# TariAgentBenchmark/unet-embroidery-seg

Measured on AMD Instinct MI355X. Metric: images/sec training unet_resnet50 512×512 bf16 at 1/2/4/8 GPUs; mIoU parity, higher is better.
Workload: dtype bf16; 1 GPU; unet_resnet50 binary seg 512x512, per-GPU batch 16, lovasz_hinge + Adam; global_batch=16, image_size=512, parallelism=dp1

## Files before the change

unet-embroidery-seg_amd/csrc/conv_fast.hip:

```cpp
#include <cstdlib>
#include <type_traits>

#include "common.h"
#include "conv_fast.h"
#include "fast_util.h"


namespace {


template <int BM, int BN, int NWM, int NWN, int ST = 3>
constexpr int tn_waves_per_simd() {
  return ST == 5 ? (BN == 64 ? 4 : 3) : (BM == 64 || (BM == 128 && BN == 64)) ? 3 : 2;
}

template <int BM, int NWM, int NWN>
constexpr int kHaloChunks() {
  constexpr int NT = 64 * NWM * NWN;
  return ((BM / 32 + 2) * 34 * 8 + 2 * NT - 1) / (2 * NT) * (2 * NT);
}
template <int BM, int BN, int NWM, int NWN, int ST, int HA = 0>
constexpr size_t kPreOff() {
  constexpr size_t stages = HA ? ((size_t)2 * kHaloChunks<BM, NWM, NWN>() + (size_t)(ST - 10) * BN * 8) * 16
                               : (size_t)(ST == 1 || ST == 5 ? 1 : ST >= 13 ? ST - 10 : 2) * (BM + BN) * 8 * 16;
// ... 615 lines not shown
  constexpr int CPR = WTN / 8;
  constexpr int RPI = 64 / CPR;
  const int ck = lane % CPR, rsub = lane / CPR;
  const int nc = n0 + wn * WTN + ck * 8;
  constexpr int NQ3 = POST == 3 ? 8 : 1;
  float q3[3][NQ3], mu3[2][NQ3], iv3[2][NQ3];
  const bool two = POST == 3 && a.aux2 != nullptr;
  if constexpr (POST == 3) {
#pragma unroll
    for (int e = 0; e < 8; ++e) {
      const bool ok = nc + e < a.Ng;
      q3[0][e] = q3[1][e] = q3[2][e] = 0.f;
      mu3[0][e] = ok ? a.pmean[nc + e] : 0.f;
      iv3[0][e] = ok ? a.pinv[nc + e] : 0.f;
      mu3[1][e] = (ok && two) ? a.pmean2[nc + e] : 0.f;
      iv3[1][e] = (ok && two) ? a.pinv2[nc + e] : 0.f;
    }
  }
  constexpr int NIT = WTM / RPI;
  constexpr int GRP = (POST == 3 && NIT > 4) ? 4 : NIT;
  static_assert(NIT % GRP == 0, "row groups");
#pragma unroll
  for (int g0 = 0; g0 < NIT; g0 += GRP) {
    uint4 oldv[GRP], zv[POST == 3 ? GRP : 1], z2v[POST == 3 ? GRP : 1];
    unsigned mkv[POST == 3 ? GRP : 1];
    if (POST == 3 || a.accumulate) {
      const bf16* aux2p = two ? (const bf16*)a.aux2 : (const bf16*)a.aux;
      const long ld2 = two ? a.ld_aux2 : a.ld_aux;
      const int ncl = nc < a.Ng ? nc : a.Ng - 8;
#pragma unroll
      for (int j = 0; j < GRP; ++j) {
        const int r = (g0 + j) * RPI + rsub;
        const long opx = out_pix(r < cnt ? row0 + r : min(row0, a.M - 1));
        oldv[j] = *reinterpret_cast<const uint4*>((const bf16*)a.y + opx * a.ldy + ncl);
        if constexpr (POST == 3) {
          zv[j] = *reinterpret_cast<const uint4*>((const bf16*)a.aux + opx * a.ld_aux + ncl);
          z2v[j] = *reinterpret_cast<const uint4*>(aux2p + opx * ld2 + ncl);
          mkv[j] = (unsigned)a.mbits[opx * (a.Ng >> 3) + (ncl >> 3)];
        }
      }
    }
#pragma unroll
    for (int j = 0; j < GRP; ++j) {
      const int r = (g0 + j) * RPI + rsub;
      if (r >= cnt || nc >= a.Ng) continue;
      const long opx = out_pix(row0 + r);
      bf16* ptr = (bf16*)a.y + opx * a.ldy + nc;
      uint4 v = *reinterpret_cast<const uint4*>(tl + r * LROW + ck * 16);
      if constexpr (POST == 3) {
        const uint4 old = oldv[j], z = zv[j], z2 = z2v[j];
        const unsigned mk = mkv[j];
        const bf16* ob = reinterpret_cast<const bf16*>(&old);
        const bf16* zb = reinterpret_cast<const bf16*>(&z);
        const bf16* z2b = reinterpret_cast<const bf16*>(&z2);
        bf16* nv = reinterpret_cast<bf16*>(&v);
#pragma unroll
        for (int e = 0; e < 8; ++e) {
          const bf16 sm = (bf16)((float)nv[e] + (float)ob[e]);
          const float d = ((mk >> e) & 1u) ? (float)sm : 0.f;
          nv[e] = (bf16)d;
          q3[0][e] += d;
          q3[1][e] = fmaf(d, ((float)zb[e] - mu3[0][e]) * iv3[0][e], q3[1][e]);
          if (two) q3[2][e] = fmaf(d, ((float)z2b[e] - mu3[1][e]) * iv3[1][e], q3[2][e]);
        }
      } else if (a.accumulate) {
        const uint4 old = oldv[j];
        const bf16* ob = reinterpret_cast<const bf16*>(&old);
        bf16* nv = reinterpret_cast<bf16*>(&v);
#pragma unroll
        for (int e = 0; e < 8; ++e) nv[e] = (bf16)((float)nv[e] + (float)ob[e]);
      }
      *reinterpret_cast<uint4*>(ptr) = v;
    }
  }
  if constexpr (POST == 3) {
#pragma unroll
    for (int q = 0; q < 3; ++q)
#pragma unroll
      for (int e = 0; e < 8; ++e)
        for (int o = CPR; o < 64; o <<= 1) q3[q][e] += __shfl_xor(q3[q][e], o, 64);
    if (rsub == 0) {
#pragma unroll
      for (int e = 0; e < 8; ++e) {
        const int col = wn * WTN + ck * 8 + e;
        red[wm * BN + col] = q3[0][e];
        red[(NWM + wm) * BN + col] = q3[1][e];
        red[(2 * NWM + wm) * BN + col] = q3[2][e];
      }
    }
  }
  if (POST) {
    const int nq = (POST == 3 && a.aux2) ? 3 : 2;
    asm volatile("s_waitcnt lgkmcnt(0)\n\ts_barrier" ::: "memory");
    for (int col = tid; col < BN; col += NT) {
      const int n = n0 + col;
      if (n >= a.Ng) continue;
      float t0 = 0.f, t1 = 0.f, t2 = 0.f;
#pragma unroll
      for (int w = 0; w < NWM; ++w) {
        t0 += red[w * BN + col];
        t1 += red[(NWM + w) * BN + col];
        if (POST == 3) t2 += red[(2 * NWM + w) * BN + col];
      }
      a.ppart[(long)tile_m * nq * a.Ng + n] = t0;
      a.ppart[(long)tile_m * nq * a.Ng + a.Ng + n] = t1;
      if (nq == 3) a.ppart[(long)tile_m * nq * a.Ng + 2 * a.Ng + n] = t2;
    }
  }
  if (a.stats) {
    asm volatile("s_waitcnt lgkmcnt(0)\n\ts_barrier" ::: "memory");
    for (int col = tid; col < BN; col += NT) {
      const int n = n0 + col;
      if (n >= a.Ng) continue;
      float st = 0.f, nt = 0.f;
#pragma unroll
      for (int w = 0; w < NWM; ++w) {
        st += red[w * BN + col];
        nt += (float)max(0, min(WTM, a.M - (m0 + w * WTM)));
      }
      const float mean = st / fmaxf(nt, 1.f);
      float q = 0.f;
#pragma unroll
      for (int w = 0; w < NWM; ++w) {
        const float nw = (float)max(0, min(WTM, a.M - (m0 + w * WTM)));
        if (nw > 0.f) {
          const float d = red[w * BN + col] / nw - mean;
          q += red[(NWM + w) * BN + col] + nw * d * d;
        }
      }
      a.stats[(long)tile_m * 2 * a.Ng + n] = st;
      a.stats[(long)tile_m * 2 * a.Ng + a.Ng + n] = q;
    }
  }
}

template <int BM, int BN, int NWM, int NWN, int ST, int POST, int TAPS = 0, bool PRE = false, int HA = 0>
__global__ __launch_bounds__(64 * NWM * NWN, (tn_waves_per_simd<BM, BN, NWM, NWN, ST>())) void tn_fast_kernel(FastTNArgs a) {
  tn_fast_body<BM, BN, NWM, NWN, ST, POST, TAPS, PRE, HA>(a, blockIdx.x + gridDim.x * blockIdx.y, gridDim.x, gridDim.y);
}

struct TNMulti {
  FastTNArgs c[4];
  int start[5];
  int gx[4], gy[4];
  int n;
};

template <int BM, int BN, int NWM, int NWN, int ST, int POST>
__global__ __launch_bounds__(64 * NWM * NWN, (tn_waves_per_simd<BM, BN, NWM, NWN>())) void tn_multi_kernel(TNMulti m) {
  const int b = blockIdx.x;
  int k = 0;
  while (k + 1 < m.n && b >= m.start[k + 1]) ++k;
  tn_fast_body<BM, BN, NWM, NWN, ST, POST, 0, false>(m.c[k], b - m.start[k], m.gx[k], m.gy[k]);
}

template <int BN, int NWN>
constexpr size_t kPersistLds() {
  constexpr int HST = kHaloChunks<256, 4, NWN>();
  return (size_t)2 * HST * 16 + (size_t)3 * BN * 8 * 16 + (size_t)2 * 4 * BN * 4;
}

template <int BN, int NWN, int POST, int HA>
__global__ __launch_bounds__(512, 2) void tn_halo_persist_kernel(FastTNArgs a, int T, int ntiles, unsigned y_bytes) {
  constexpr int BM = 256, NWM = 4, NT = 512, NS = 3;
  constexpr int WTN = BN / NWN, FP = 4, FC = WTN / 16;
  constexpr int RSTEP = NT / 8;
  constexpr int B_PER = BN / RSTEP;
  static_assert(B_PER == 1 || B_PER == 2, "weight rows per thread");
  constexpr int HST = kHaloChunks<BM, NWM, NWN>();
  constexpr int HI = HST / NT;
  constexpr int HPIX = 10 * 34;
  constexpr int WST = BN * 8;
  constexpr int WP = B_PER;
  constexpr int HPC = HI / HA, TPER = 9 / HA;
  static_assert(HI % (2 * HA) == 0 && 9 % HA == 0, "halo pieces of whole instruction pairs");
  constexpr int NST = FC * FP;
  static_assert(WP + 2 * HPC + NST + 2 <= 63, "vmcnt range");
  extern __shared__ __attribute__((aligned(16))) uint4 lds[];

  const int tid = threadIdx.x, lane = tid & 63;
  const int wid = __builtin_amdgcn_readfirstlane(tid >> 6);
  const int wm = wid / NWN, wn = wid % NWN;
  const int kv = tid & 7, rb = tid >> 3;
  const int kg = lane >> 4, j16 = lane & 15;
  const int gy = (a.Ng + BN - 1) / BN;
  const int tpr = a.wc >> 5;
  const int nch = a.cin >> 6;

  const unsigned hbase = lds_addr(lds);
  const unsigned wbase = hbase + 2u * HST * 16u;
  float* red = reinterpret_cast<float*>(reinterpret_cast<char*>(lds) + 2 * HST * 16 + 3 * WST * 16);
  float* xco = red + 2 * NWM * BN;
  const bool has_bias = a.bias != nullptr;
  if (has_bias)
    for (int c = tid; c < a.Ng; c += NT) xco[c] = a.bias[c];
  if (POST && a.post == 2)
    for (int c = tid; c < a.Ng; c += NT) {
      xco[c] = a.psc[c];
      xco[a.Ng + c] = a.psh[c];
      xco[2 * a.Ng + c] = a.pmean[c];
      xco[3 * a.Ng + c] = a.pinv[c];
    }
  __syncthreads();

  const int nbk = gridDim.x, b = blockIdx.x;
  const int xq = nbk >> 3, xr = nbk & 7, xcd = b & 7;
  const int lb = (xcd < xr ? xcd * (xq + 1) : xr * (xq + 1) + (xcd - xr) * xq) + (b >> 3);
  const int tfirst = lb * T;
  const int tcount = max(0, min(T, ntiles - tfirst));

  const unsigned pb1 = a.x1_bytes / (unsigned)a.ldc1b;
  const unsigned pb2 = a.x2 ? a.x2_bytes / (unsigned)a.ldc2b : 0u;
  const unsigned pbad = (pb1 > pb2 ? pb1 : pb2) + 1u;
  const unsigned hsw = (unsigned)(((lane & 7) ^ ((lane >> 3) & 7)) * 16);
  const int kvs16 = (kv ^ ((rb >> 1) & 7)) * 16;
  struct Tile {
    int tm, n0, nb, h0, w0;
  };
  auto tile_of = [&](int j) -> Tile {
    const int tl = tfirst + j;
    Tile t;
    t.tm = tl / gy;
    t.n0 = (tl - t.tm * gy) * BN;
    const int rest = t.tm / tpr, twi = t.tm - rest * tpr;
    const int hg = rest * 8;
    t.nb = hg / a.hc;
    t.h0 = hg - t.nb * a.hc;
    t.w0 = twi * 32;
    return t;
  };
  auto halo_pix = [&](const Tile& t, int i) -> unsigned {
    const int hp = (i * (NWM * NWN) + wid) * 8 + (lane >> 3);
    const int hr = hp / 34, hc = hp - hr * 34;
    const int h = t.h0 - 1 + hr, w = t.w0 - 1 + hc;
    const bool ok = hp < HPIX && h >= 0 && h < a.H && w >= 0 && w < a.W;
    return ok ? (unsigned)((t.nb * a.H + h) * a.W + w) : pbad;
  };
  auto wrow = [&](const Tile& t, int i) -> unsigned {
    const int n = t.n0 + rb + RSTEP * i;
    return n < a.Ng ? (unsigned)n * (unsigned)a.ldwb + kvs16 : kOOB;
  };
  unsigned tw[9];
#pragma unroll
  for (int t = 0; t < 9; ++t) {
    const int jr = t / 3, js = t - jr * 3;
    tw[t] = (unsigned)(((a.r0 + a.rs * jr) * a.S + (a.s0 + a.ss * js)) * a.cin) * 2u;
  }
  int hq[FP];
#pragma unroll
  for (int p = 0; p < FP; ++p) hq[p] = (wm * 2 + (p >> 1) + 1) * 34 + (p & 1) * 16 + j16 + 1;
  const int chA = kg;
  unsigned foffW[2];
#pragma unroll
  for (int kk = 0; kk < 2; ++kk) {
    const int r = j16;
    foffW[kk] = (unsigned)((wn * WTN + r) * 128 + ((kk * 4 + kg) ^ ((r >> 1) & 7)) * 16);
  }
  auto issue_halo = [&](const Tile& tt, bool live, int cc, int hs, int i0, int i1) {
    const int c64 = cc * 64;
    const bool first = c64 < a.c1;
    const __amdgpu_buffer_rsrc_t rx = srd_u(first ? a.x1 : a.x2, !live ? 0u : first ? a.x1_bytes : a.x2_bytes);
    const unsigned ldcb = first ? (unsigned)a.ldc1b : (unsigned)a.ldc2b;
    const unsigned soff = __builtin_amdgcn_readfirstlane(live ? (unsigned)(first ? c64 : c64 - a.c1) * 2u : 0u);
    const unsigned sb = __builtin_amdgcn_readfirstlane(hbase + (unsigned)(hs * HST * 16) + (unsigned)(wid * 1024));
#pragma unroll
    for (int i = i0; i < i1; i += 2)
      dma16x2<NT * 16>(rx, sb + (unsigned)(i * NT * 16), __umul24(halo_pix(tt, i), ldcb) + hsw,
                       __umul24(halo_pix(tt, i + 1), ldcb) + hsw, soff);
  };
  auto issue_w = [&](const Tile& tt, bool live, int cc, int t, int stage) {
    const __amdgpu_buffer_rsrc_t rwx = srd_u(a.wt, live ? a.w_bytes : 0u);
    const unsigned wsoff = __builtin_amdgcn_readfirstlane(live ? tw[t] + (unsigned)(cc * 64) * 2u : 0u);
    const unsigned sb = __builtin_amdgcn_readfirstlane(wbase + (unsigned)(stage * WST * 16) + (unsigned)(wid * 8 * 128));
    if constexpr (B_PER == 1) {
      dma16s(rwx, sb, wrow(tt, 0), wsoff);
    } else {
      dma16x2<RSTEP * 128>(rwx, sb, wrow(tt, 0), wrow(tt, 1), wsoff);
    }
  };
  constexpr auto P_ = [](int t) { return ((((t % 9) + 9) % 9) % TPER == 0) ? HPC : 0; };

  const __amdgpu_buffer_rsrc_t ry = srd(a.y, y_bytes);
  const bool do_stats = a.stats != nullptr;
  const __amdgpu_buffer_rsrc_t raux = srd(POST ? a.aux : a.y, POST ? (unsigned)a.M * (unsigned)a.ld_aux * 2u : 0u);
  const __amdgpu_buffer_rsrc_t rq = srd(POST ? (const void*)a.ppart : do_stats ? (const void*)a.stats : a.y,
                                        (POST || do_stats) ? (unsigned)(a.M / BM) * 2u * (unsigned)a.Ng * 4u : 0u);
  const int E = NST + ((POST || do_stats) ? 2 : 0);

  if (tcount <= 0) return;
  Tile cur = tile_of(0);
  issue_halo(cur, true, 0, 0, 0, HI);
  issue_w(cur, true, 0, 0, 0);
  issue_w(cur, true, 0, 1, 1);

  int gc = 0;
  for (int j = 0; j < tcount; ++j) {
    const bool has_next = j + 1 < tcount;
    const Tile nxt = has_next ? tile_of(j + 1) : cur;
    f32x4 acc[FC][FP];
#pragma unroll
    for (int c = 0; c < FC; ++c)
#pragma unroll
      for (int p = 0; p < FP; ++p) acc[c][p] = f32x4{0.f, 0.f, 0.f, 0.f};
    uint2 zr[FC][FP];
    unsigned opix[FP];
#pragma unroll
// ... 515 lines not shown

template <int BM, int BN, int NWM, int NWN, int ST>
static int launch_tn_dma(const FastTNArgs& a, hipStream_t st) {
  switch (tn_taps(a)) {
    case 9: return a.post ? launch_tn_cfg<BM, BN, NWM, NWN, ST, true, 9>(a, st) : launch_tn_cfg<BM, BN, NWM, NWN, ST, false, 9>(a, st);
    case 1: return a.post ? launch_tn_cfg<BM, BN, NWM, NWN, ST, true, 1>(a, st) : launch_tn_cfg<BM, BN, NWM, NWN, ST, false, 1>(a, st);
    default: return a.post ? launch_tn_cfg<BM, BN, NWM, NWN, ST, true>(a, st) : launch_tn_cfg<BM, BN, NWM, NWN, ST>(a, st);
  }
}

static bool halo_a_ok(const FastTNArgs& a) {
  if (getenv("UNETSEG_TN_NO_HALO_RING") != nullptr || a.in_sc || a.nr != 3 || a.ns != 3 || a.istride != 1) return false;
  if (a.dhs * a.dhs != 1 || a.dws * a.dws != 1) return false;
  const int dh_lo = a.dhs > 0 ? a.dh0 : a.dh0 - 2, dw_lo = a.dws > 0 ? a.dw0 : a.dw0 - 2;
  if (dh_lo != -1 || dw_lo != -1) return false;
  if (a.H != a.hc || a.W != a.wc || a.hc % 8 || a.wc % 32) return false;
  return tn_taps(a) == 9;
}

static int tn_config_base(const FastTNArgs& a);

static int cu_count() {
  static int n = 0;
  if (!n) {
    int dev = 0;
    if (hipGetDevice(&dev) != hipSuccess || hipDeviceGetAttribute(&n, hipDeviceAttributeMultiprocessorCount, dev) != hipSuccess ||
        n <= 0)
      n = 256;
  }
  return n;
}
static int persist_t(const FastTNArgs& a, int bn) {
  const char* e = getenv("UNETSEG_TN_PERSIST");
  if (e && atoi(e) == 0) return 0;
  if (a.in_sc || a.post < 0 || a.post > 2 || (a.bias && a.post) || a.t2d < 0) return 0;
  if (a.ostride != 1 || a.ph || a.pw || a.OH != a.hc || a.OW != a.wc || a.M % 256) return 0;
  const size_t extra = (a.bias ? (size_t)a.Ng * 4 : 0) + (a.post == 2 ? (size_t)a.Ng * 16 : 0);
  const size_t lds = (bn == 128 ? kPersistLds<128, 2>() : kPersistLds<64, 2>()) + extra;
  if (lds > 160 * 1024) return 0;
  if ((unsigned long long)a.M * (unsigned)a.ldy * 2ull >= (unsigned long long)kOOB) return 0;
  if (a.post && (unsigned long long)a.M * (unsigned)a.ld_aux * 2ull >= (unsigned long long)kOOB) return 0;
  if (a.stats && (unsigned long long)(a.M / 256) * 2ull * a.Ng * 4ull >= (unsigned long long)kOOB) return 0;
  const char* mc = getenv("UNETSEG_TN_PERSIST_MIN_NCH");
  if (mc && (a.cin >> 6) < atoi(mc)) return 0;
  const long ntiles = (long)(a.M / 256) * ceil_div(a.Ng, bn);
  const char* ft = getenv("UNETSEG_TN_PERSIST_T");
  if (ft && atoi(ft) > 0) return atoi(ft);
  const char* r = getenv("UNETSEG_TN_PERSIST_ROUNDS");
  const int rounds = r && atoi(r) > 0 ? atoi(r) : 1;
  const char* m = getenv("UNETSEG_TN_PERSIST_MIN_T");
  const int min_t = m && atoi(m) > 0 ? atoi(m) : 2;
  const long T = (ntiles + (long)rounds * cu_count() - 1) / ((long)rounds * cu_count());
  return T >= min_t ? (int)T : 0;
}

template <int BN, int NWN, int HA>
static int launch_tn_persist(const FastTNArgs& a, hipStream_t st) {
  const int T = persist_t(a, BN);
  const size_t extra = (a.bias ? (size_t)a.Ng * 4 : 0) + (a.post == 2 ? (size_t)a.Ng * 16 : 0);
  const size_t lds = kPersistLds<BN, NWN>() + extra;
  const int ntiles = (a.M / 256) * ceil_div(a.Ng, BN);
  const int grid = ceil_div(ntiles, T);
  const unsigned y_bytes = (unsigned)((unsigned long long)a.M * (unsigned)a.ldy * 2ull);
  if (a.post) {
    static bool attr = false;
    if (!attr) {
      (void)hipFuncSetAttribute(reinterpret_cast<const void*>(&tn_halo_persist_kernel<BN, NWN, 1, HA>),
                                hipFuncAttributeMaxDynamicSharedMemorySize, 160 * 1024);
      attr = true;
    }
    hipLaunchKernelGGL((tn_halo_persist_kernel<BN, NWN, 1, HA>), dim3(grid), dim3(512), lds, st, a, T, ntiles, y_bytes);
  } else {
    static bool attr = false;
    if (!attr) {
      (void)hipFuncSetAttribute(reinterpret_cast<const void*>(&tn_halo_persist_kernel<BN, NWN, 0, HA>),
                                hipFuncAttributeMaxDynamicSharedMemorySize, 160 * 1024);
      attr = true;
    }
    hipLaunchKernelGGL((tn_halo_persist_kernel<BN, NWN, 0, HA>), dim3(grid), dim3(512), lds, st, a, T, ntiles, y_bytes);
  }
  return 0;
}

static int tn_config(const FastTNArgs& a) {
  if (a.force_cfg) return a.force_cfg;
  const int c = tn_config_base(a);
  if ((c == 7 || c == 13 || (c == 10 && !getenv("UNETSEG_TN_CFG_NO23"))) && halo_a_ok(a)) return c == 7 ? 21 : c == 13 ? 22 : 23;
  return c;
}

static int tn_config_base(const FastTNArgs& a) {
  if (const char* e = getenv("UNETSEG_TN_CFG")) {
    const int c = atoi(e);
    if (c == 21) return 7;
    if (((c >= 1 && c <= 14) || c == 19 || c == 20) && !(a.in_sc && c >= 7 && c <= 14)) return c;
  }
  static const bool no_dma_env = getenv("UNETSEG_TN_NO_DMA") != nullptr;
  const bool no_dma = no_dma_env || a.in_sc != nullptr;
  if (!a.in_sc && halo3_ok(a)) return 0;
  const int nsteps = a.nr * a.ns * (a.cin >> 6);
  static const bool no_short1 = getenv("UNETSEG_TN_NO_SHORT1") != nullptr;
  if (!no_short1 && nsteps <= 4 && (nsteps >= 2 || a.Ng <= 64)) return a.Ng <= 64 ? 20 : 19;
  if (nsteps == 1 && a.Ng > 64) return 4;
  if (a.Ng <= 64) return (!no_dma && nsteps >= 18 && tn_taps(a) == 9) ? 13 : 6;
  if (nsteps <= 4) return 3;
  const long tiles_big = (long)ceil_div(a.M, 256) * ceil_div(a.Ng, 128);
  if (tiles_big >= 256) return no_dma ? 2 : 7;
  const long tiles_mid = (long)ceil_div(a.M, 128) * ceil_div(a.Ng, 128);
  if (tiles_mid >= 256) return (!no_dma && nsteps >= 16 && tn_taps(a)) ? 10 : 3;
  return (!no_dma && nsteps >= 32) ? 9 : 5;
}

}

static int tn_cfg_bm(int cfg) {
  switch (cfg) {
    case 1: case 2: case 7: case 11: case 14: case 21: case 22: return 256;
    case 23: return 128;
    case 5: case 9: return 64;
    default: return 128;
  }
}

bool tn_fast_ok(const FastTNArgs& a) {
  return a.cin % 64 == 0 && a.c1 % 64 == 0 && a.nr * a.ns <= 32 && a.Ng % 8 == 0;
}

int tn_fast_tile_m(const FastTNArgs& a) {
  const int cfg = tn_config(a);
  return cfg == 0 ? halo_tile_m() : tn_cfg_bm(cfg);
}

int tn_fast_post_rows(const FastTNArgs& a) {
  if (a.M <= 0 || a.Ng <= 0) return 0;
  const int cfg = tn_config(a);
  return cfg == 0 ? halo3_blocks(a) : ceil_div(a.M, tn_cfg_bm(cfg));
}

int tn_fast_config(const FastTNArgs& a, int* taps_out) {
  const int cfg = tn_config(a);
  if ((cfg == 21 || cfg == 22) && !a.in_sc && a.post != 3 && a.post != 4 && persist_t(a, cfg == 21 ? 128 : 64) > 0) {
    if (taps_out) *taps_out = 0;
    return cfg + 3;
  }
  if (taps_out) *taps_out = (cfg >= 7 && cfg <= 14) ? tn_taps(a) : 0;
  return cfg;
}

bool tn_fast_post_res_ok(const FastTNArgs& a) {
  const int cfg = tn_config(a);
  return cfg == 4 || cfg == 19 || cfg == 20 || ((cfg == 7 || cfg == 10) && tn_taps(a) == 1);
}

static int launch_tn_post_res(const FastTNArgs& a, hipStream_t st) {
  switch (tn_config(a)) {
    case 4: return launch_tn_cfg<128, 128, 2, 2, 1, 3>(a, st);
    case 19: return launch_tn_cfg<128, 128, 2, 2, 5, 3>(a, st);
    case 20: return launch_tn_cfg<128, 64, 2, 2, 5, 3>(a, st);
    case 7: return tn_taps(a) == 1 ? launch_tn_cfg<256, 128, 4, 2, 13, 3, 1>(a, st) : -1;
    case 10: return tn_taps(a) == 1 ? launch_tn_cfg<128, 128, 2, 2, 15, 3, 1>(a, st) : -1;
    default: return -1;
  }
}

int launch_tn_fast(const FastTNArgs& a, hipStream_t st) {
  if (a.M <= 0 || a.Ng <= 0) return 0;
  if (a.post == 3) return a.in_sc ? -1 : launch_tn_post_res(a, st);
  if (a.post == 4) return tn_config(a) == 0 ? launch_halo3(a, st) : -1;
  if (a.in_sc) {
    switch (tn_config(a)) {
      case 1: return launch_tn_cfg<256, 64, 4, 1, 2, false, 0, true>(a, st);
      case 2: return launch_tn_cfg<256, 128, 4, 2, 3, false, 0, true>(a, st);
      case 4: return launch_tn_cfg<128, 128, 2, 2, 1, false, 0, true>(a, st);
      case 5: return launch_tn_cfg<64, 128, 1, 4, 3, false, 0, true>(a, st);
      case 6: return launch_tn_cfg<128, 64, 2, 2, 3, false, 0, true>(a, st);
      case 3: return launch_tn_cfg<128, 128, 2, 2, 3, false, 0, true>(a, st);
      case 19: return launch_tn_cfg<128, 128, 2, 2, 5, false, 0, true>(a, st);
      case 20: return launch_tn_cfg<128, 64, 2, 2, 5, false, 0, true>(a, st);
      default: return -1;
    }
  }
  switch (tn_config(a)) {
    case 0: return launch_halo3(a, st);
    case 1: return a.post ? launch_tn_cfg<256, 64, 4, 1, 2, true>(a, st) : launch_tn_cfg<256, 64, 4, 1, 2>(a, st);
    case 2: return a.post ? launch_tn_cfg<256, 128, 4, 2, 3, true>(a, st) : launch_tn_cfg<256, 128, 4, 2, 3>(a, st);
    case 4: return a.post ? launch_tn_cfg<128, 128, 2, 2, 1, true>(a, st) : launch_tn_cfg<128, 128, 2, 2, 1>(a, st);
    case 5: return a.post ? launch_tn_cfg<64, 128, 1, 4, 3, true>(a, st) : launch_tn_cfg<64, 128, 1, 4, 3>(a, st);
    case 6: return a.post ? launch_tn_cfg<128, 64, 2, 2, 3, true>(a, st) : launch_tn_cfg<128, 64, 2, 2, 3>(a, st);
    case 7: return launch_tn_dma<256, 128, 4, 2, 13>(a, st);
    case 8: return launch_tn_dma<128, 128, 2, 2, 14>(a, st);
    case 9: return launch_tn_dma<64, 128, 1, 4, 14>(a, st);
    case 10: return launch_tn_dma<128, 128, 2, 2, 15>(a, st);
    case 11: return launch_tn_dma<256, 64, 4, 1, 13>(a, st);
    case 12: return launch_tn_dma<128, 64, 2, 2, 14>(a, st);
    case 13: return launch_tn_dma<128, 64, 2, 2, 13>(a, st);
    case 14: return launch_tn_dma<256, 64, 4, 2, 13>(a, st);
    case 19: return a.post ? launch_tn_cfg<128, 128, 2, 2, 5, true>(a, st) : launch_tn_cfg<128, 128, 2, 2, 5>(a, st);
    case 20: return a.post ? launch_tn_cfg<128, 64, 2, 2, 5, true>(a, st) : launch_tn_cfg<128, 64, 2, 2, 5>(a, st);
    case 21: {
      if (persist_t(a, 128) > 0) return launch_tn_persist<128, 2, 3>(a, st);
      static const bool ns4 = getenv("UNETSEG_TN_HALO_NS4") != nullptr;
      static const bool split = !(getenv("UNETSEG_TN_HALO_SPLIT") && atoi(getenv("UNETSEG_TN_HALO_SPLIT")) == 1);
      if (ns4) return a.post ? launch_tn_cfg<256, 128, 4, 2, 14, true, 9, false, 1>(a, st)
                             : launch_tn_cfg<256, 128, 4, 2, 14, false, 9, false, 1>(a, st);
      if (split) return a.post ? launch_tn_cfg<256, 128, 4, 2, 13, true, 9, false, 3>(a, st)
                               : launch_tn_cfg<256, 128, 4, 2, 13, false, 9, false, 3>(a, st);
      return a.post ? launch_tn_cfg<256, 128, 4, 2, 13, true, 9, false, 1>(a, st)
                    : launch_tn_cfg<256, 128, 4, 2, 13, false, 9, false, 1>(a, st);
    }
    case 22:
      if (persist_t(a, 64) > 0) return launch_tn_persist<64, 2, 1>(a, st);
      return a.post ? launch_tn_cfg<256, 64, 4, 2, 13, true, 9, false, 1>(a, st)
                           : launch_tn_cfg<256, 64, 4, 2, 13, false, 9, false, 1>(a, st);
    case 23: return a.post ? launch_tn_cfg<128, 128, 2, 2, 15, true, 9, false, 1>(a, st)
                           : launch_tn_cfg<128, 128, 2, 2, 15, false, 9, false, 1>(a, st);
    default: return a.post ? launch_tn_cfg<128, 128, 2, 2, 3, true>(a, st) : launch_tn_cfg<128, 128, 2, 2, 3>(a, st);
  }
}

static bool tn_multi_off() {
  static const bool off = getenv("UNETSEG_NO_TN_MULTI") != nullptr;
  return off;
}

int tn_multi_tile_m(const FastTNArgs* fs, int n) {
  if (tn_multi_off() || n < 2 || n > 4) return -1;
  bool bm64 = false;
  for (int k = 0; k < n; ++k) {
    if (fs[k].in_sc || fs[k].M <= 0) return -1;
    const int cfg = tn_config(fs[k]);
    if (cfg == 0) return -1;
    if (tn_cfg_bm(cfg) == 64) bm64 = true;
  }
  return bm64 ? 64 : 128;
}

int launch_tn_multi(const FastTNArgs* fs, int n, hipStream_t st) {
  const int bm = tn_multi_tile_m(fs, n);
  if (bm < 0) return -1;
  const bool post = fs[0].post != 0;
  if (bm == 64) return post ? launch_tn_multi_cfg<64, 128, 1, 4, 3, true>(fs, n, st)
                            : launch_tn_multi_cfg<64, 128, 1, 4, 3, false>(fs, n, st);
  return post ? launch_tn_multi_cfg<128, 128, 2, 2, 3, true>(fs, n, st)
              : launch_tn_multi_cfg<128, 128, 2, 2, 3, false>(fs, n, st);
}

bool wgrad_fast_ok(const FastWgradArgs& a) {
  return a.cin % 8 == 0 && a.c1 % 8 == 0 && a.Cout % 64 == 0;
}

int wgrad_fast_splits(int Cout, int Ng, long Kpix) {
  const int bm = Cout <= 64 ? 64 : 128;
  const int bn = Cout <= 64 ? 256 : 128;
  const int tiles = ceil_div(Cout, bm) * ceil_div(Ng, bn);
  const long nkt = (Kpix + kWgBK - 1) / kWgBK;
  static const int wscale = getenv("UNETSEG_WG_BLOCKS") ? atoi(getenv("UNETSEG_WG_BLOCKS")) : 256;
  int sp = ceil_div(wscale > 0 ? wscale : (Cout <= 64 ? 1024 : 512), tiles);
  const long max_sp = nkt / 32 > 0 ? nkt / 32 : 1;
  if (sp > max_sp) sp = (int)max_sp;
  if (sp > 512) sp = 512;
  if (sp < 1) sp = 1;
  return sp;
}

template <int BM, int BN, int NWM, int NWN, bool ROW32, bool PRE = false>
static void launch_wgrad_cfg(const FastWgradArgs& a, int splits, hipStream_t st) {
  const size_t lds = 2 * (size_t)kWgBK * (BM / 8 + BN / 8) * 16;
  static bool attr = false;
  if (!attr) {
    (void)hipFuncSetAttribute(reinterpret_cast<const void*>(&wgrad_fast_kernel<BM, BN, NWM, NWN, ROW32, PRE>),
                              hipFuncAttributeMaxDynamicSharedMemorySize, (int)lds);
    attr = true;
  }
  dim3 grid(ceil_div(a.Cout, BM), ceil_div(a.Ng, BN), splits);
  hipLaunchKernelGGL((wgrad_fast_kernel<BM, BN, NWM, NWN, ROW32, PRE>), grid, dim3(64 * NWM * NWN), lds, st, a);
}

int wgrad_fast_kind(const FastWgradArgs& a) {
  const bool small = a.Cout <= 64;
  if (wgrad_ring_ok(a)) return small ? kWgRing64x256 : kWgRing128;
  static const bool no_row = getenv("UNETSEG_WG_NO_ROW32") != nullptr;
  const bool row32 = !no_row && a.Q % kWgBK == 0;
  return small ? (row32 ? kWgFastRow64x256 : kWgFast64x256) : (row32 ? kWgFastRow128 : kWgFast128);
}

template <bool PRE>
static void launch_wgrad_kind(int kind, const FastWgradArgs& a, int splits, hipStream_t st) {
  switch (kind) {
    case kWgFastRow64x256: return launch_wgrad_cfg<64, 256, 1, 4, true, PRE>(a, splits, st);
    case kWgFast64x256: return launch_wgrad_cfg<64, 256, 1, 4, false, PRE>(a, splits, st);
    case kWgFastRow128: return launch_wgrad_cfg<128, 128, 2, 2, true, PRE>(a, splits, st);
    default: return launch_wgrad_cfg<128, 128, 2, 2, false, PRE>(a, splits, st);
  }
}

int launch_wgrad_fast(FastWgradArgs a, int splits, hipStream_t st) {
  const long nkt = (a.Kpix + kWgBK - 1) / kWgBK;
  a.kt_per_split = (int)((nkt + splits - 1) / splits);
  const int kind = wgrad_fast_kind(a);
  if (kind == kWgRing64x256 || kind == kWgRing128) return launch_wgrad_ring(a, splits, st);
  if (a.in_sc) launch_wgrad_kind<true>(kind, a, splits, st);
  else launch_wgrad_kind<false>(kind, a, splits, st);
  return 0;
}
```

Measured before the change: 1017 images/s.

## Add persistent weight-resident streaming kernel for 1x1 residual-post convolutions

Adds a persistent kernel for 1x1 convolutions with the residual post-op (post==3) and input channels up to 256. Each block loads its 128-column weight slice into LDS once and then walks many 128-row M tiles, double-buffering activations through registers. The fused epilogue does the residual add, masking and per-channel partial statistics. The aim is to stop reloading weights for every tile and to cut launch and tail overhead on grids with many tiles. The cost is large LDS use, which limits occupancy, plus a new code path whose numerical results must match the existing tiled kernels.

```diff
diff --git a/unet-embroidery-seg_amd/csrc/conv_fast.hip b/unet-embroidery-seg_amd/csrc/conv_fast.hip
--- a/unet-embroidery-seg_amd/csrc/conv_fast.hip
+++ b/unet-embroidery-seg_amd/csrc/conv_fast.hip
@@ -791,6 +791,216 @@
   int k = 0;
   while (k + 1 < m.n && b >= m.start[k + 1]) ++k;
   tn_fast_body<BM, BN, NWM, NWN, ST, POST, 0, false>(m.c[k], b - m.start[k], m.gx[k], m.gy[k]);
+}
+
+constexpr int kStreamWork = 4 * 64 * (64 * 2 + 16) + 3 * 2 * 128 * 4;
+constexpr size_t stream_lds(int nch) { return (size_t)kStreamWork + (size_t)nch * 128 * 128 + 4 * 128 * 4; }
+
+template <int NCH, bool TWO>
+__global__ __launch_bounds__(256, (NCH <= 2 ? 2 : 1)) void tn_stream_post3_kernel(FastTNArgs a, int gy, int rs, int ntm) {
+  constexpr int BM = 128, BN = 128, NWM = 2, NWN = 2, NT = 256;
+  constexpr int WTM = 64, WTN = 64, FP = 4, FC = 4, RSTEP = 32, A_PER = 4, B_PER = 4;
+  static_assert(kStreamWork >= 2 * BM * 128 && kStreamWork % 16 == 0, "two A stages inside the epilogue scratch");
+  extern __shared__ __attribute__((aligned(16))) uint4 lds[];
+  uint4* const Wl = lds + kStreamWork / 16;
+  float* const coef = reinterpret_cast<float*>(Wl + NCH * BN * 8);
+
+  const int tid = threadIdx.x, lane = tid & 63;
+  const int wid = __builtin_amdgcn_readfirstlane(tid >> 6);
+  const int wm = wid / NWN, wn = wid % NWN;
+  const int xcd = blockIdx.x & 7, jx = blockIdx.x >> 3;
+  const int tile_n = jx % gy;
+  const int tm0 = xcd * rs + jx / gy, tstep = 8 * rs;
+  if (tm0 >= ntm) return;
+  const int n0 = tile_n * BN;
+  const int kv = tid & 7, rb = tid >> 3;
+
+  const __amdgpu_buffer_rsrc_t r1 = srd(a.x1, a.x1_bytes);
+  const __amdgpu_buffer_rsrc_t rw = srd(a.wt, a.w_bytes);
+
+  {
+    const unsigned wtap = (unsigned)((a.r0 * a.S + a.s0) * a.cin) * 2u;
+    uint4 wv[NCH][B_PER];
+#pragma unroll
+    for (int kt = 0; kt < NCH; ++kt)
+#pragma unroll
+      for (int i = 0; i < B_PER; ++i)
+        wv[kt][i] = bload(rw, (unsigned)(n0 + rb + RSTEP * i) * (unsigned)a.ldwb + kv * 16 + wtap + kt * 128);
+#pragma unroll
+    for (int kt = 0; kt < NCH; ++kt)
+#pragma unroll
+      for (int i = 0; i < B_PER; ++i) {
+        const int row = rb + RSTEP * i;
+        Wl[kt * BN * 8 + row * 8 + swz8(row, kv)] = wv[kt][i];
+      }
+    if (tid < BN) {
+      coef[tid] = a.pmean[n0 + tid];
+      coef[BN + tid] = a.pinv[n0 + tid];
+      coef[2 * BN + tid] = TWO ? a.pmean2[n0 + tid] : 0.f;
+      coef[3 * BN + tid] = TWO ? a.pinv2[n0 + tid] : 0.f;
+    }
+  }
+
+  uint4 ra[NCH][A_PER];
+  auto load_a = [&](int tm) {
+#pragma unroll
+    for (int i = 0; i < A_PER; ++i) {
+      const int m = tm * BM + rb + RSTEP * i;
+      const unsigned off = (tm < ntm && m < a.M) ? (unsigned)m * (unsigned)a.ldc1b + kv * 16 : kOOB;
+#pragma unroll
+      for (int kt = 0; kt < NCH; ++kt) ra[kt][i] = bload(r1, off == kOOB ? kOOB : off + kt * 128);
+    }
+  };
+  auto store_a = [&](int buf, const uint4 (&v)[A_PER]) {
+    uint4* L = lds + buf * (BM * 8);
+#pragma unroll
+    for (int i = 0; i < A_PER; ++i) {
+      const int row = rb + RSTEP * i;
+      L[row * 8 + swz8(row, kv)] = v[i];
+    }
+  };
+  unsigned foffA[2], foffB[2];
+#pragma unroll
+  for (int kk = 0; kk < 2; ++kk) {
+    const int r = lane & 15, sw = ((kk * 4 + (lane >> 4)) ^ ((r >> 1) & 7)) * 16;
+    foffA[kk] = (unsigned)((wm * WTM + r) * 128 + sw);
+    foffB[kk] = (unsigned)((wn * WTN + r) * 128 + sw);
+  }
+
+  const int kg = lane >> 4, j16 = lane & 15;
+  constexpr int LROW = WTN * 2 + 16;
+  char* const tl = reinterpret_cast<char*>(lds) + wid * (WTM * LROW);
+  float* const red = reinterpret_cast<float*>(reinterpret_cast<char*>(lds) + NWM * NWN * WTM * LROW);
+  constexpr int CPR = WTN / 8, RPI = 64 / CPR, NIT = WTM / RPI;
+  const int ck = lane % CPR, rsub = lane / CPR;
+  const int nc = n0 + wn * WTN + ck * 8;
+  const float* const cf = coef + wn * WTN + ck * 8;
+  constexpr int nq = TWO ? 3 : 2;
+
+  uint4 oldv[NIT], zv[NIT], z2v[TWO ? NIT : 1];
+  unsigned mkv[NIT];
+  auto load_aux = [&](int tm) {
+    const int row0 = tm * BM + wm * WTM;
+    const int cnt = min(WTM, a.M - row0);
+#pragma unroll
+    for (int j = 0; j < NIT; ++j) {
+      const int r = j * RPI + rsub;
+      const long opx = r < cnt ? row0 + r : min(row0, a.M - 1);
+      oldv[j] = *reinterpret_cast<const uint4*>((const bf16*)a.y + opx * a.ldy + nc);
+      zv[j] = *reinterpret_cast<const uint4*>((const bf16*)a.aux + opx * a.ld_aux + nc);
+      if constexpr (TWO) z2v[j] = *reinterpret_cast<const uint4*>((const bf16*)a.aux2 + opx * a.ld_aux2 + nc);
+      mkv[j] = (unsigned)a.mbits[opx * (a.Ng >> 3) + (nc >> 3)];
+    }
+  };
+
+  load_a(tm0);
+  for (int tm = tm0; tm < ntm; tm += tstep) {
+    const int m0 = tm * BM;
+    f32x4 acc[FC][FP];
+#pragma unroll
+    for (int c = 0; c < FC; ++c)
+#pragma unroll
+      for (int p = 0; p < FP; ++p) acc[c][p] = f32x4{0.f, 0.f, 0.f, 0.f};
+
+    store_a(0, ra[0]);
+    asm volatile("s_waitcnt lgkmcnt(0)\n\ts_barrier" ::: "memory");
+#pragma unroll
+    for (int kt = 0; kt < NCH; ++kt) {
+      if (kt + 1 < NCH) store_a((kt + 1) & 1, ra[kt + 1]);
+      const char* sa = reinterpret_cast<const char*>(lds + (kt & 1) * (BM * 8));
+      const char* sb = reinterpret_cast<const char*>(Wl + kt * BN * 8);
+#pragma unroll
+      for (int kk = 0; kk < 2; ++kk) {
+        bf16x8 pf[FP], wf[FC];
+#pragma unroll
+        for (int p = 0; p < FP; ++p) pf[p] = *reinterpret_cast<const bf16x8*>(sa + foffA[kk] + p * 2048);
+#pragma unroll
+        for (int c = 0; c < FC; ++c) wf[c] = *reinterpret_cast<const bf16x8*>(sb + foffB[kk] + c * 2048);
+#pragma unroll
+        for (int c = 0; c < FC; ++c)
+#pragma unroll
+          for (int p = 0; p < FP; ++p)
+            acc[c][p] = __builtin_amdgcn_mfma_f32_16x16x32_bf16(wf[c], pf[p], acc[c][p], 0, 0, 0);
+      }
+      asm volatile("s_waitcnt lgkmcnt(0)\n\ts_barrier" ::: "memory");
+    }
+
+    load_a(tm + tstep);
+
+    const int row0 = m0 + wm * WTM;
+    const int cnt = min(WTM, a.M - row0);
+#pragma unroll
+    for (int p = 0; p < FP; ++p) {
+      const bool mok = p * 16 + j16 < cnt;
+#pragma unroll
+      for (int c = 0; c < FC; ++c) {
+        bf16 ob[4];
+#pragma unroll
+        for (int e = 0; e < 4; ++e) {
+          const float v = acc[c][p][e] + 0.f;
+          ob[e] = (bf16)(mok ? (float)(bf16)v : 0.f);
+        }
+        *reinterpret_cast<uint2*>(tl + (p * 16 + j16) * LROW + (c * 16 + kg * 4) * 2) = *reinterpret_cast<uint2*>(ob);
+      }
+    }
+    load_aux(tm);
+    __builtin_amdgcn_s_waitcnt(0xC07F);
+    __builtin_amdgcn_wave_barrier();
+    float q3[3][8];
+#pragma unroll
+    for (int e = 0; e < 8; ++e) q3[0][e] = q3[1][e] = q3[2][e] = 0.f;
+#pragma unroll
+    for (int j = 0; j < NIT; ++j) {
+      const int r = j * RPI + rsub;
+      if (r >= cnt) continue;
+      bf16* ptr = (bf16*)a.y + (long)(row0 + r) * a.ldy + nc;
+      uint4 v = *reinterpret_cast<const uint4*>(tl + r * LROW + ck * 16);
+      const uint4 old = oldv[j], z = zv[j], z2 = TWO ? z2v[j] : zv[j];
+      const unsigned mk = mkv[j];
+      const bf16* ob = reinterpret_cast<const bf16*>(&old);
+      const bf16* zb = reinterpret_cast<const bf16*>(&z);
+      const bf16* z2b = reinterpret_cast<const bf16*>(&z2);
+      bf16* nv = reinterpret_cast<bf16*>(&v);
+#pragma unroll
+      for (int e = 0; e < 8; ++e) {
+        const bf16 sm = (bf16)((float)nv[e] + (float)ob[e]);
+        const float d = ((mk >> e) & 1u) ? (float)sm : 0.f;
+        nv[e] = (bf16)d;
+        q3[0][e] += d;
+        q3[1][e] = fmaf(d, ((float)zb[e] - cf[e]) * cf[BN + e], q3[1][e]);
+        if (TWO) q3[2][e] = fmaf(d, ((float)z2b[e] - cf[2 * BN + e]) * cf[3 * BN + e], q3[2][e]);
+      }
+      *reinterpret_cast<uint4*>(ptr) = v;
+    }
+#pragma unroll
+    for (int q = 0; q < 3; ++q)
+#pragma unroll
+      for (int e = 0; e < 8; ++e)
+        for (int o = CPR; o < 64; o <<= 1) q3[q][e] += __shfl_xor(q3[q][e], o, 64);
+    if (rsub == 0) {
+#pragma unroll
+      for (int e = 0; e < 8; ++e) {
+        const int col = wn * WTN + ck * 8 + e;
+        red[wm * BN + col] = q3[0][e];
+        red[(NWM + wm) * BN + col] = q3[1][e];
+        red[(2 * NWM + wm) * BN + col] = q3[2][e];
+      }
+    }
+    asm volatile("s_waitcnt lgkmcnt(0)\n\ts_barrier" ::: "memory");
+    if (tid < BN) {
+      const int col = tid, n = n0 + col;
+      float t0 = 0.f, t1 = 0.f, t2 = 0.f;
+#pragma unroll
+      for (int w = 0; w < NWM; ++w) {
+        t0 += red[w * BN + col];
+        t1 += red[(NWM + w) * BN + col];
+        t2 += red[(2 * NWM + w) * BN + col];
+      }
+      a.ppart[(long)tm * nq * a.Ng + n] = t0;
+      a.ppart[(long)tm * nq * a.Ng + a.Ng + n] = t1;
+      if (nq == 3) a.ppart[(long)tm * nq * a.Ng + 2 * a.Ng + n] = t2;
+    }
+  }
 }
 
 template <int BN, int NWN>
@@ -1612,8 +1822,55 @@
   return cfg == 4 || cfg == 19 || cfg == 20 || ((cfg == 7 || cfg == 10) && tn_taps(a) == 1);
 }
 
+static int post3_stream_rs(const FastTNArgs& a) {
+  const char* e = getenv("UNETSEG_POST3_STREAM");
+  if (e && atoi(e) == 0) return 0;
+  if (a.post != 3 || a.in_sc || a.bias || a.relu || a.stats || a.x2 || a.c1 != a.cin || a.force_cfg) return 0;
+  if (a.nr != 1 || a.ns != 1 || a.dh0 || a.dw0 || a.istride != 1 || a.ostride != 1 || a.ph || a.pw) return 0;
+  if (a.OH != a.hc || a.OW != a.wc || a.H != a.hc || a.W != a.wc) return 0;
+  if (a.cin % 64 || a.cin > 256 || a.Ng % 128 || a.M <= 0) return 0;
+  if ((unsigned long long)a.M * (unsigned)a.ldc1b >= (unsigned long long)kOOB) return 0;
+  const int nch = a.cin >> 6, gy = a.Ng / 128, ntm = ceil_div(a.M, 128);
+  const int by_lds = (int)((size_t)160 * 1024 / stream_lds(nch)), by_regs = nch <= 2 ? 2 : 1;
+  int blocks = cu_count() * (by_lds < by_regs ? by_lds : by_regs);
+  const char* mb = getenv("UNETSEG_POST3_STREAM_MAXB");
+  if (mb && atoi(mb) > 0 && atoi(mb) < blocks) blocks = atoi(mb);
+  int rs = blocks / (8 * gy);
+  if (rs < 1) rs = 1;
+  if (rs > ceil_div(ntm, 8)) rs = ceil_div(ntm, 8);
+  return rs;
+}
+
+template <int NCH, bool TWO>
+static int launch_tn_stream_cfg(const FastTNArgs& a, int rs, hipStream_t st) {
+  static bool attr = false;
+  if (!attr) {
+    (void)hipFuncSetAttribute(reinterpret_cast<const void*>(&tn_stream_post3_kernel<NCH, TWO>),
+                              hipFuncAttributeMaxDynamicSharedMemorySize, (int)stream_lds(NCH));
+    attr = true;
+  }
+  const int gy = a.Ng / 128;
+  hipLaunchKernelGGL((tn_stream_post3_kernel<NCH, TWO>), dim3(8 * gy * rs), dim3(256), stream_lds(NCH), st, a, gy, rs,
+                     ceil_div(a.M, 128));
+  return 0;
+}
+
+static int launch_tn_stream(const FastTNArgs& a, int rs, hipStream_t st) {
+  const bool two = a.aux2 != nullptr;
+  switch (a.cin >> 6) {
+    case 1: return two ? launch_tn_stream_cfg<1, true>(a, rs, st) : launch_tn_stream_cfg<1, false>(a, rs, st);
+    case 2: return two ? launch_tn_stream_cfg<2, true>(a, rs, st) : launch_tn_stream_cfg<2, false>(a, rs, st);
+    case 3: return two ? launch_tn_stream_cfg<3, true>(a, rs, st) : launch_tn_stream_cfg<3, false>(a, rs, st);
+    case 4: return two ? launch_tn_stream_cfg<4, true>(a, rs, st) : launch_tn_stream_cfg<4, false>(a, rs, st);
+    default: return -1;
+  }
+}
+
 static int launch_tn_post_res(const FastTNArgs& a, hipStream_t st) {
-  switch (tn_config(a)) {
+  const int cfg = tn_config(a);
+  if (cfg == 4 || cfg == 19)
+    if (const int rs = post3_stream_rs(a)) return launch_tn_stream(a, rs, st);
+  switch (cfg) {
     case 4: return launch_tn_cfg<128, 128, 2, 2, 1, 3>(a, st);
     case 19: return launch_tn_cfg<128, 128, 2, 2, 5, 3>(a, st);
     case 20: return launch_tn_cfg<128, 64, 2, 2, 5, 3>(a, st);
```

Result: no change. 1023 images/s, median of 6 (+0.6%).
